# domargan/parallel-packed-csr

Hardware: AMD Instinct MI355X
Metric: edge-updates/sec (higher is better)
Workload: dtype u32; 1 GPU; config#2 1000000 random inserts on RMAT scale-20 / 10000000-edge core, 1 partition, labels raw; vertices=1048576, core_edges=10000000, parallelism=1 partition(s), 1 per GPU x 1 GPU(s), logN=32, distinct_update_batches=4, semantics=sequential stream order (bit-exact vs reference -threads=1)

## Files before the change

parallel-packed-csr_amd/csrc/engine.cc:

```cpp
#include "engine.h"

#include <stdio.h>
#include <stdlib.h>

#include <algorithm>
#include <map>
#include <memory>
#include <vector>
#include <chrono>

#include "gpu_rt.h"
#define GPU_DFREE(x) gpu::dfree_named((x), #x, __LINE__)
#include "pma_kernels.h"

namespace ppcsr {

#define GCHK(expr)                                                                       \
  do {                                                                                   \
    int _e = (expr);                                                                     \
    if (_e != 0) return fail(PPCSR_EHIP, std::string(#expr) + ": " + gpu::err_str(_e)); \
  } while (0)

struct DevGuard {
  std::vector<void **> slots;
// ... 41 lines not shown
  ChainTable *d_table = nullptr;
  unsigned long long *d_scan_state = nullptr;
  uint64_t scan_state_cap = 0, scan_nchunks = 0;
  Edge *d_scratch = nullptr;
  uint64_t scratch_cap = 0;
  int *d_nbr = nullptr;
  uint64_t nbr_cap = 0;
  uint32_t round = 0;
  uint32_t max_horizon = 4096, min_horizon = 64, rounds_per_sync = 32, init_horizon = 256;
  gpu::Timer timer;
  EngineStats st{};
  struct Snap {
    View v{};
    uint64_t cap_slots = 0, cap_nodes = 0;
    bool valid = false;
    uint32_t synced = 0;
    uint64_t gen = 0;
  };
  Snap snap, esnap;
  uint32_t snap_grid = 4096;
  bool snap_count = false;
  uint64_t snap_ctr[6] = {0, 0, 0, 0, 0, 0};
  unsigned long long *d_snapcnt = nullptr;
  uint64_t scc_ctr[8] = {0, 0, 0, 0, 0, 0, 0, 0};
  uint64_t msf_ctr[8] = {0, 0, 0, 0, 0, 0, 0, 0};
  uint32_t serial = 1;
  uint64_t array_gen = 1;
  bool stamps_clean = false;
  OptCtl *d_octl = nullptr, *h_octl = nullptr;
  uint32_t *d_vdbg = nullptr;
  uint32_t *d_status = nullptr, *d_carry0 = nullptr, *d_carry1 = nullptr;
  uint64_t carry_cap = 0, hslot_cap = 0;
  unsigned long long *d_regfail = nullptr, *d_pfail = nullptr;
  uint32_t *d_vws = nullptr, *d_vrs = nullptr;
  uint32_t *d_wstamp = nullptr, *d_rstamp = nullptr;
  uint32_t mode = 1;
  uint32_t epoch_ops = 1u << 20;
  uint32_t cur_epoch = 0;
  uint32_t epoch_short = 16384;
  uint32_t epoch_clean = 0, epoch_grow_after = 2;
  uint32_t epoch_adapt = 8, grow_eff = 2;
  uint64_t since_rollback = 0;
  double rb_dist = -1.0;
  uint32_t region_slots = 1024;
  uint32_t region_wide = 4096, region_calm = 8, region_eff = 0, region_clean = 0;
  uint32_t region_rare = 16384, region_rare_calm = 8, region_rare_dist = 65536;
  uint64_t region_rare_span = 0;
  uint32_t region_rare_cpr = 1536;
  double cpr_mean = -1.0;
  uint32_t resident_waves = 0;
  uint32_t opt_horizon = 6144;
  uint32_t start_horizon = 6144;
  uint32_t adaptive = 1;
  uint32_t rb_defer_table = 1u << 22;
  uint32_t scatter_blocks = 8192;
  uint32_t small_batch = 256;
  uint32_t excl_in_wave = 4096;
  uint32_t big_window = 32768, big_min = 256, big_grid = 64;
  dev::BigJob *d_jobs = nullptr;
  Edge *d_bigscratch = nullptr;
  uint64_t bigscratch_cap = 0;
  uint32_t rb_tile = 0;
  uint32_t rb_min_tiles = 4096;
  bool big_on = false;
  double big_rate = 0;
  bool check_lanes = true;
  uint32_t check_wave_chunks = 0;
  int check_force = -1;
  uint32_t rb_prefetch = 1;
  bool time_resize = false;
  double last_resize_ms = 0;
  uint32_t rb_bench_upper = 0;
  uint64_t rb_inplace_min = 1ull << 19;
  uint32_t rb_inplace_cpw = 0;
  uint32_t *d_ip = nullptr;
  uint32_t ip_epoch = 0;
  uint32_t ip_lists = 1;
  bool ip_used = false;
  uint32_t scatter_variant = 2;
  bool partial = false;
  bool profile = false;
  bool in_batch = false;
  uint32_t soft_barrier = 0;
  uint32_t defer_barrier = 0;
  uint32_t dbg_repeat = 0;
  uint32_t diag = 0;
// ... 12 lines not shown
    uint64_t rows_cap = 0;
    uint32_t *crow = nullptr, *ccnt = nullptr;
    unsigned long long *ooff = nullptr;
    uint64_t chunk_cap = 0;
    int *sdst = nullptr;
    uint32_t *sval = nullptr;
    uint64_t stage_cap = 0;
    unsigned long long *xs = nullptr;
    uint64_t xs_cap = 0;
  } q;
};

Engine::Engine() : p_(new Impl()) {}

static int ensure_plans(Engine::Impl &p) {
  const uint64_t need = (uint64_t)std::max(p.opt_horizon, p.max_horizon) + 64;
  if (p.plans_cap >= need) return 0;
  int e = gpu::sync(p.stream);
  if (e) return e;
  Plan *np = nullptr;
  if ((e = gpu::dmalloc((void **)&np, need * sizeof(Plan)))) return e;
  if (p.d_plans) GPU_DFREE(p.d_plans);
  p.d_plans = np;
  p.plans_cap = need;
  return 0;
}

static int reset_tags(Engine::Impl &p) {
  const uint64_t leaves = p.v.g.N >> p.v.g.sh;
  int e;
  if (p.v.wres && (e = gpu::dset(p.v.wres, 0xFF, leaves * sizeof(unsigned long long), p.stream))) return e;
  if (p.v.rres && (e = gpu::dset(p.v.rres, 0xFF, leaves * sizeof(unsigned long long), p.stream))) return e;
  if (p.v.dres && (e = gpu::dset(p.v.dres, 0xFF, leaves * sizeof(unsigned long long), p.stream))) return e;
  if (p.d_regfail && (e = gpu::dset(p.d_regfail, 0xFF, (leaves + 1) * sizeof(unsigned long long), p.stream))) return e;
  if (p.d_pfail && (e = gpu::dset(p.d_pfail, 0xFF, (leaves + 1) * sizeof(unsigned long long), p.stream))) return e;
  if (p.v.vw && (e = gpu::dset(p.v.vw, 0xFF, (p.n_cap + 1) * sizeof(unsigned long long), p.stream))) return e;
  if (p.v.vr && (e = gpu::dset(p.v.vr, 0xFF, (p.n_cap + 1) * sizeof(unsigned long long), p.stream))) return e;
  p.round = 0;
  return 0;
}

static int alloc_aux(Engine::Impl &p, View &v) {
  const uint64_t leaves = v.g.N >> v.g.sh;
  int e;
  if ((e = gpu::dmalloc((void **)&v.wres, leaves * sizeof(unsigned long long)))) return e;
  if ((e = gpu::dmalloc((void **)&v.rres, leaves * sizeof(unsigned long long)))) return e;
  if ((e = gpu::dmalloc((void **)&v.dres, leaves * sizeof(unsigned long long)))) return e;
  if ((e = gpu::dset(v.dres, 0xFF, leaves * sizeof(unsigned long long), p.stream))) return e;
  if ((e = gpu::dmalloc((void **)&p.d_wstamp, leaves * sizeof(uint32_t)))) return e;
  if ((e = gpu::dmalloc((void **)&p.d_rstamp, leaves * sizeof(uint32_t)))) return e;
  if ((e = gpu::dmalloc((void **)&p.d_regfail, (leaves + 1) * sizeof(unsigned long long)))) return e;
  if ((e = gpu::dmalloc((void **)&p.d_pfail, (leaves + 1) * sizeof(unsigned long long)))) return e;
  if ((e = gpu::dset(p.d_pfail, 0xFF, (leaves + 1) * sizeof(unsigned long long), p.stream))) return e;
  if ((e = gpu::dset(v.wres, 0xFF, leaves * sizeof(unsigned long long), p.stream))) return e;
  if ((e = gpu::dset(v.rres, 0xFF, leaves * sizeof(unsigned long long), p.stream))) return e;
  if ((e = gpu::dset(p.d_regfail, 0xFF, (leaves + 1) * sizeof(unsigned long long), p.stream))) return e;
  if ((e = gpu::dset(p.d_wstamp, 0, leaves * sizeof(uint32_t), p.stream))) return e;
  if ((e = gpu::dset(p.d_rstamp, 0, leaves * sizeof(uint32_t), p.stream))) return e;
  if ((e = gpu::dmalloc((void **)&v.ldirty, leaves * sizeof(uint32_t)))) return e;
  if ((e = gpu::dset(v.ldirty, 0, leaves * sizeof(uint32_t), p.stream))) return e;
  p.leaves_cap = leaves;
  p.round = 0;
  if (v.vw && (e = gpu::dset(v.vw, 0xFF, (p.n_cap + 1) * sizeof(unsigned long long), p.stream))) return e;
  if (v.vr && (e = gpu::dset(v.vr, 0xFF, (p.n_cap + 1) * sizeof(unsigned long long), p.stream))) return e;
  return 0;
}
static int alloc_vertex_aux(Engine::Impl &p, View &v) {
  const uint64_t cap = p.n_cap + 1;
  int e;
  if (v.vw) GPU_DFREE(v.vw);
  if (v.vr) GPU_DFREE(v.vr);
  if (p.d_vws) GPU_DFREE(p.d_vws);
  if (p.d_vrs) GPU_DFREE(p.d_vrs);
  if (v.vdirty) GPU_DFREE(v.vdirty);
  v.vw = v.vr = nullptr;
  v.vdirty = nullptr;
  p.d_vws = p.d_vrs = nullptr;
  if ((e = gpu::dmalloc((void **)&v.vdirty, cap * sizeof(uint32_t)))) return e;
  if ((e = gpu::dset(v.vdirty, 0, cap * sizeof(uint32_t), p.stream))) return e;
  if ((e = gpu::dmalloc((void **)&v.vw, cap * sizeof(unsigned long long)))) return e;
  if ((e = gpu::dmalloc((void **)&v.vr, cap * sizeof(unsigned long long)))) return e;
// ... 40 lines not shown
}

int Engine::create(uint32_t init_n, uint32_t src_n, int lock_search, int device, Engine **out, std::string *errmsg) {
  Engine *e = new Engine();
  int rc = e->init(init_n, src_n, lock_search, device);
  if (rc != PPCSR_OK) {
    if (errmsg) *errmsg = e->err_;
    e->p_->partial = true;
    delete e;
    *out = nullptr;
    return rc;
  }
  *out = e;
  return PPCSR_OK;
}

int Engine::init(uint32_t init_n, uint32_t src_n, int lock_search, int device) {
  Impl &p = *p_;
  device_ = device;
  int ndev = 0;
  GCHK(gpu::device_count(&ndev));
  if (ndev <= 0) return fail(PPCSR_EHIP, "no HIP device visible: the MI355X engine has no CPU fallback");
  if (device < 0 || device >= ndev) return fail(PPCSR_EINVAL, "bad device ordinal");
  GCHK(gpu::set_device(device));
  (void)gpu::last_error();
  GCHK(gpu::stream_create(&p.stream));
  GCHK(p.timer.init());
  {
    int cus = 0;
    GCHK(gpu::device_cus(device, &cus));
    if (cus > 0) {
      p.resident_waves = (uint32_t)cus * 28u;
      p.start_horizon = p.resident_waves;
      p.opt_horizon = 3u * p.resident_waves;
    }
  }
  const uint64_t N = initial_N(init_n, src_n);
  Geometry g;
  compute_geometry(N, src_n, lock_search, &g);
  p.v.g = g;
  p.v.big_window = kBigWindow;
  p.v.serial = p.serial;
  p.n_cap = std::max<uint64_t>(src_n, 16);
  p.leaves_cap = N >> g.sh;
  GCHK(gpu::dmalloc((void **)&p.v.items, N * sizeof(Edge)));
  GCHK(gpu::dmalloc((void **)&p.v.nodes, p.n_cap * sizeof(Node)));
  GCHK(gpu::dmalloc((void **)&p.v.leafcnt, p.leaves_cap * sizeof(uint32_t)));
  GCHK(alloc_aux(p, p.v));
  GCHK(alloc_vertex_aux(p, p.v));
  GCHK(gpu::dmalloc((void **)&p.d_octl, sizeof(OptCtl)));
  GCHK(gpu::hmalloc((void **)&p.h_octl, sizeof(OptCtl)));
  GCHK(gpu::dmalloc((void **)&p.d_ctl, sizeof(Control)));
  GCHK(gpu::hmalloc((void **)&p.h_ctl, sizeof(Control)));
  GCHK(gpu::dmalloc((void **)&p.d_stats, kStatShards * sizeof(StatShard)));
  GCHK(gpu::hmalloc((void **)&p.h_stats, kStatShards * sizeof(StatShard)));
  GCHK(gpu::dset(p.d_stats, 0, kStatShards * sizeof(StatShard), p.stream));
  GCHK(gpu::dmalloc((void **)&p.d_stats_snap, kStatShards * sizeof(StatShard)));
  GCHK(gpu::dmalloc((void **)&p.d_xout, sizeof(ExclOut)));
  GCHK(gpu::hmalloc((void **)&p.h_xout, sizeof(ExclOut)));
  GCHK(gpu::hmalloc((void **)&p.h_op1, sizeof(Op)));
  GCHK(gpu::dmalloc((void **)&p.d_total, 32 * sizeof(unsigned long long)));
  GCHK(gpu::hmalloc((void **)&p.h_total, sizeof(unsigned long long)));
  GCHK(gpu::dmalloc((void **)&p.d_table, sizeof(ChainTable)));
  GCHK(gpu::dmalloc((void **)&p.d_ip, (kIpHdrWords + 2 * (uint64_t)kIpMaxTiles) * sizeof(uint32_t)));
  GCHK(gpu::dset(p.d_ip, 0, (kIpHdrWords + 2 * (uint64_t)kIpMaxTiles) * sizeof(uint32_t), p.stream));
  {
    uint32_t *probe = p.d_ip + kIpHdrWords;
// ... 19 lines not shown

  std::vector<Node> nodes(src_n);
  {
    double index_d = 0.0;
    const double step = ((double)N) / src_n;
    for (uint32_t i = 0; i < src_n; i++) {
      nodes[i].beginning = (i == 0) ? 0u : nodes[i - 1].end;
      index_d += step;
      nodes[i].end = (uint32_t)(int)index_d;
      nodes[i].num_neighbors = 0;
    }
    if (src_n != 0) nodes[src_n - 1].end = (uint32_t)(N - 1);
  }
  if (src_n) {
    GCHK(gpu::h2d(p.v.nodes, nodes.data(), (uint64_t)src_n * sizeof(Node), p.stream));
    GCHK(gpu::sync(p.stream));
  }
  GPU_LAUNCH(p.stream, k_fill_null, grid_for(N * 3, 256 * 8), 256, p.v.items, (uint64_t)0, N);
  if (src_n) GPU_LAUNCH(p.stream, k_place_sentinels, grid_for(src_n, 256), 256, p.v);
  GPU_LAUNCH(p.stream, k_recount, grid_for((N + 63) / 64, 4), 256, p.v, (uint64_t)0, N);
  GCHK(gpu::sync(p.stream));
  GCHK(gpu::last_error());
  return PPCSR_OK;
}

Engine::~Engine() {
  Impl &p = *p_;
  gpu::set_device(device_);
  gpu::sync(p.stream);
  GPU_DFREE(p.v.items);
  GPU_DFREE(p.v.nodes);
  GPU_DFREE(p.v.leafcnt);
  free_aux(p, p.v);
  if (p.v.vw) GPU_DFREE(p.v.vw);
  if (p.v.vr) GPU_DFREE(p.v.vr);
  if (p.d_vws) GPU_DFREE(p.d_vws);
  if (p.d_vrs) GPU_DFREE(p.d_vrs);
  if (p.v.vdirty) GPU_DFREE(p.v.vdirty);
  GPU_DFREE(p.d_octl);
  gpu::hfree(p.h_octl);
  if (p.d_status) GPU_DFREE(p.d_status);
  if (p.d_vdbg) GPU_DFREE(p.d_vdbg);
  if (p.d_carry0) GPU_DFREE(p.d_carry0);
  if (p.d_carry1) GPU_DFREE(p.d_carry1);
  GPU_DFREE(p.d_ctl);
  gpu::hfree(p.h_ctl);
  GPU_DFREE(p.d_stats);
  gpu::hfree(p.h_stats);
  GPU_DFREE(p.d_stats_snap);
  GPU_DFREE(p.d_xout);
  gpu::hfree(p.h_xout);
  gpu::hfree(p.h_op1);
  GPU_DFREE(p.d_total);
  gpu::hfree(p.h_total);
  GPU_DFREE(p.d_table);
  if (p.d_ip) GPU_DFREE(p.d_ip);
  if (p.d_snapcnt) GPU_DFREE(p.d_snapcnt);
  GPU_DFREE(p.d_plans);
  if (p.d_ops) GPU_DFREE(p.d_ops);
  if (p.d_rank) GPU_DFREE(p.d_rank);
  if (p.d_tiles) GPU_DFREE(p.d_tiles);
  if (p.d_nbr) GPU_DFREE(p.d_nbr);
  if (p.d_scratch) GPU_DFREE(p.d_scratch);
  if (p.d_scan_state) GPU_DFREE(p.d_scan_state);
  if (p.d_jobs) GPU_DFREE(p.d_jobs);
  if (p.d_bigscratch) GPU_DFREE(p.d_bigscratch);
// ... 48 lines not shown
  if (k == "region_slots") {
    if (value < 1 || (value & (value - 1))) return fail(PPCSR_EINVAL, "region_slots must be a power of two");
    p.region_slots = (uint32_t)value;
    p.region_eff = 0;
    return PPCSR_OK;
  }
  if (k == "region_wide") {
    if (value < 1 || (value & (value - 1))) return fail(PPCSR_EINVAL, "region_wide must be a power of two");
    p.region_wide = (uint32_t)value;
    return PPCSR_OK;
  }
  if (k == "region_rare") {
    if (value < 0 || (value & (value - 1))) return fail(PPCSR_EINVAL, "region_rare must be 0 or a power of two");
    p.region_rare = (uint32_t)value;
    return PPCSR_OK;
  }
  if (k == "region_rare_calm") {
    p.region_rare_calm = (uint32_t)std::max<int64_t>(1, value);
    return PPCSR_OK;
  }
  if (k == "region_rare_cpr") {
    p.region_rare_cpr = (uint32_t)std::max<int64_t>(0, value);
    return PPCSR_OK;
  }
  if (k == "region_rare_dist") {
    p.region_rare_dist = (uint32_t)std::max<int64_t>(1, value);
    return PPCSR_OK;
  }
  if (k == "region_calm") {
    p.region_calm = (uint32_t)std::max<int64_t>(1, value);
    return PPCSR_OK;
  }
  if (k == "opt_horizon") {
    if (value < 1 || value > (1 << 20)) return fail(PPCSR_EINVAL, "opt_horizon out of range");
    p.opt_horizon = (uint32_t)value;
    gpu::set_device(device_);
    GCHK(ensure_plans(p));
    p.start_horizon = std::min<uint32_t>(p.start_horizon, p.opt_horizon);
    if (!p.adaptive) p.start_horizon = p.opt_horizon;
    return PPCSR_OK;
  }
  if (k == "scatter_blocks") {
    p.scatter_blocks = (uint32_t)std::max<int64_t>(64, value);
    return PPCSR_OK;
  }
  if (k == "search_narrow") {
    p.v.g.narrow = value ? 1u : 0u;
    return PPCSR_OK;
  }
  if (k == "small_batch") {
    p.small_batch = value < 0 ? 0u : (uint32_t)value;
    return PPCSR_OK;
  }
  if (k == "excl_in_wave") {
    p.excl_in_wave = (uint32_t)std::max<int64_t>(64, value);
    return PPCSR_OK;
  }
  if (k == "big_window") {
    if (value < 64 || (value & (value - 1))) return fail(PPCSR_EINVAL, "big_window must be a power of two >= 64");
    p.big_window = (uint32_t)std::min<int64_t>(value, 1 << 20);
    return PPCSR_OK;
  }
  if (k == "big_min") {
    p.big_min = (uint32_t)std::max<int64_t>(64, std::min<int64_t>(value, kBigWindow));
    return PPCSR_OK;
  }
  if (k == "big_grid") {
    p.big_grid = (uint32_t)std::max<int64_t>(1, std::min<int64_t>(value, 256));
    return PPCSR_OK;
  }
  if (k == "rb_tile") {
    uint32_t t = 0;
    if (value > 0) for (t = 8; t < (uint32_t)value && t < kRbTile; t <<= 1) {}
    p.rb_tile = t;
// ... 21 lines not shown
    p.snap_grid = (uint32_t)value;
    return PPCSR_OK;
  }
  if (k == "snap_count") {
    if (value && !p.d_snapcnt) {
      gpu::set_device(device_);
      GCHK(gpu::dmalloc((void **)&p.d_snapcnt, 2 * sizeof(unsigned long long)));
    }
    p.snap_count = value != 0;
    return PPCSR_OK;
  }
  if (k == "rb_inplace_cpw") {
    p.rb_inplace_cpw = value >= 16 ? 16u : (value >= 8 ? 8u : 0u);
    return PPCSR_OK;
  }
  if (k == "rb_inplace_min") {
    p.rb_inplace_min = value < 0 ? 0ull : (uint64_t)value;
    return PPCSR_OK;
  }
  if (k == "check_lanes") {
    p.check_force = value < 0 ? -1 : (value ? 1 : 0);
    return PPCSR_OK;
  }
  if (k == "rb_bench_upper") {
    p.rb_bench_upper = value ? 1u : 0u;
    return PPCSR_OK;
  }
  if (k == "rb_prefetch") {
    p.rb_prefetch = value ? 1u : 0u;
    return PPCSR_OK;
  }
  if (k == "scatter_variant") {
    p.scatter_variant = value > 2 ? 2u : (uint32_t)value;
    return PPCSR_OK;
  }
  if (k == "adaptive") {
    p.adaptive = value != 0;
    return PPCSR_OK;
  }
  if (k == "resident_waves") {
    if (value < 0 || value > (1 << 20)) return fail(PPCSR_EINVAL, "resident_waves out of range");
    p.resident_waves = (uint32_t)value;
    return PPCSR_OK;
  }
  if (k == "start_horizon") {
    if (value < 1 || value > (1 << 20)) return fail(PPCSR_EINVAL, "start_horizon out of range");
    p.start_horizon = (uint32_t)value;
    return PPCSR_OK;
  }
  if (k == "test_block_rebalance") {
    const uint64_t ws = (uint64_t)value >> 32, wl = (uint64_t)value & 0xFFFFFFFFull;
    if (wl < 64 || (wl & (wl - 1)) || ws % wl || ws + wl > p.v.g.N || (wl >> p.v.g.sh) > dev::kBigLeaves) return fail(PPCSR_EINVAL, "bad window");
    gpu::set_device(device_);
    Edge *sc = nullptr;
    GCHK(gpu::dmalloc((void **)&sc, wl * sizeof(Edge)));
    GPU_LAUNCH(p.stream, k_block_rebalance, 1, dev::kBigThreads, p.v, ws, wl, sc);
    GCHK(gpu::sync(p.stream));
    GCHK(gpu::last_error());
    gpu::dfree(sc);
    return PPCSR_OK;
  }
  if (k == "marker") {
    gpu::set_device(device_);
    uint32_t *np_ = nullptr;
    switch (value) {
      case 0: GPU_LAUNCH(p.stream, k_mark_0, 1, 64, np_); break;
// ... 253 lines not shown
  const uint32_t kEpochShort = p.epoch_short;
  if (p.cur_epoch == 0 || p.cur_epoch > p.epoch_ops) p.cur_epoch = p.epoch_ops;
  while (e0 < n) {
    uint64_t e1 = std::min<uint64_t>(e0 + p.cur_epoch, n);
    if (forced_e1 > e0 && forced_e1 < e1) e1 = forced_e1;
    if (p.round > 0xFFFF0000u) GCHK(reset_tags(p));
    GCHK(snap_commit(p, p.esnap));
    GCHK(gpu::d2d(p.d_stats_snap, p.d_stats, kStatShards * sizeof(StatShard), p.stream));
    if (!p.stamps_clean) {
      const uint64_t leaves = p.v.g.N >> p.v.g.sh;
      GCHK(gpu::dset(p.d_wstamp, 0, leaves * sizeof(uint32_t), p.stream));
      GCHK(gpu::dset(p.d_rstamp, 0, leaves * sizeof(uint32_t), p.stream));
      GCHK(gpu::dset(p.d_vws, 0, (p.n_cap + 1) * sizeof(uint32_t), p.stream));
      GCHK(gpu::dset(p.d_vrs, 0, (p.n_cap + 1) * sizeof(uint32_t), p.stream));
      p.stamps_clean = true;
    }
    OptCtl &c = *p.h_octl;
    memset(&c, 0, sizeof(c));
    const uint32_t pp0 = p.round & 1u;
    c.hor[pp0] = 0;
    c.used[pp0] = 0;
    c.nf[pp0] = (uint32_t)e0;
    c.adaptive = p.adaptive;
    c.cur_h[pp0] = p.adaptive ? std::min(p.start_horizon, p.opt_horizon) : p.opt_horizon;
    c.book_round = p.round;
    for (int t = 0; t < 3; t++) {
      c.minkept[t] = kMax;
      c.gbar[t] = c.sbar[t] = ~0ull;
    }
    c.e1 = (uint32_t)e1;
    c.max_horizon = p.opt_horizon;
    c.width_cap = p.opt_horizon;
    c.resident = p.resident_waves;
    c.viol_idx = kMax;
    c.skip_idx = kMax;
    c.skip_round = 0;
    GCHK(gpu::h2d(p.d_octl, p.h_octl, sizeof(OptCtl), p.stream));
    int rs = 0;
    if (p.region_eff < p.region_slots) p.region_eff = p.region_slots;
    while ((p.region_eff >> rs) > (uint32_t)p.v.g.logN) rs++;
    bool epoch_open = true;
    uint32_t cur_width = c.cur_h[pp0];
    uint64_t carry_now = 0;
    unsigned long long jobs_seen = 0, rounds_seen = 0, planned_seen = 0, long_seen = 0;
    uint64_t chunk_pending = e1 - e0;
    double chunk_cpr = 0.9 * (double)std::min<uint64_t>(cur_width, e1 - e0);
    unsigned long long prev_rounds = 0, prev_committed = 0;
    uint32_t excl_cooldown = 0;
    while (epoch_open) {
      OptArgs a;
      a.v = p.v;
      a.v.big_window = use_big ? bigw : kBigWindow;
      a.big_min = p.big_min;
      a.jobs = use_big ? p.d_jobs : (dev::BigJob *)nullptr;
      a.bigscratch = p.d_bigscratch;
      a.bigscratch_stride = bigw;
      a.ops = d_ops;
      a.plans = p.d_plans;
      a.status = p.d_status;
      a.vdbg = p.d_vdbg;
      a.carry0 = p.d_carry0;
      a.carry1 = p.d_carry1;
      a.carry_cap = (uint32_t)p.carry_cap;
      a.ctl = p.d_octl;
      a.stats = p.d_stats;
      a.regfail = p.d_regfail;
      a.pfail = p.d_pfail;
      a.wstamp = p.d_wstamp;
      a.rstamp = p.d_rstamp;
      a.vws = p.d_vws;
      a.vrs = p.d_vrs;
      a.regshift = rs;
      a.diag = p.diag;
      a.defer_barrier = p.defer_barrier;
      const bool extras = p.diag != 0 || p.dbg_repeat != 0;
      a.dbg = p.dbg_repeat;
      a.dg = p.diag >= 2 ? p.d_dg : (uint32_t *)nullptr;
      a.soft_barrier = p.soft_barrier ? p.soft_barrier : a.v.big_window / 2u;
      if (!p.soft_barrier && p.region_rare_span && p.region_eff >= p.region_rare) a.soft_barrier = 0x40000000u;
      uint32_t gh = p.opt_horizon;
      {
        const uint64_t want = std::max<uint64_t>(1024, 4ull * (cur_width ? cur_width : p.opt_horizon));
        if (want < gh) gh = (uint32_t)want;
        const uint64_t pend = (chunk_pending + 255) & ~255ull;
        if (pend < gh) gh = (uint32_t)std::max<uint64_t>(pend, 256);
        const uint64_t need = (carry_now + 255) & ~255ull;
        if (gh < need) gh = (uint32_t)std::min<uint64_t>(need, p.opt_horizon);
      }
      const uint32_t blocks = (gh + 3) / 4;
      if (gh != c.max_horizon) {
        GCHK(gpu::h2d(&p.d_octl->max_horizon, &gh, sizeof(uint32_t), p.stream));
        c.max_horizon = gh;
      }
      uint32_t rounds = p.rounds_per_sync;
      {
        const double per_round = std::max(1.0, 0.85 * chunk_cpr);
        const double est = (double)chunk_pending / per_round + 2.0;
        if (est < (double)rounds) rounds = (uint32_t)std::max(2.0, est);
      }
      if (excl_cooldown) {
        rounds = std::min<uint32_t>(rounds, 8u);
        excl_cooldown--;
      }
      if (p.profile && p.events.size() < 5ull * rounds) {
        const size_t oldn = p.events.size();
        p.events.resize(5ull * rounds);
        for (size_t i = oldn; i < p.events.size(); i++) GCHK(p.events[i].init());
      }
      for (uint32_t r = 0; r < rounds; r++) {
        a.round = ++p.round;
        if (p.profile) p.events[5 * r + 0].record(p.stream);
        if (extras) GPU_LAUNCH(p.stream, o_plan_x, blocks, 256, a); else GPU_LAUNCH(p.stream, o_plan, blocks, 256, a);
        if (p.profile) p.events[5 * r + 1].record(p.stream);
        if (extras) GPU_LAUNCH(p.stream, o_check_x, blocks, 256, a);
        else if (p.check_force >= 0 ? p.check_force == 1 : p.check_lanes) GPU_LAUNCH(p.stream, o_check, (gh + kCkThreads - 1) / kCkThreads, kCkThreads, a);
        else GPU_LAUNCH(p.stream, o_check_w, blocks, 256, a);
        if (p.profile) p.events[5 * r + 2].record(p.stream);
        if (extras) GPU_LAUNCH(p.stream, o_apply_x, blocks, 256, a); else GPU_LAUNCH(p.stream, o_apply, blocks, 256, a);
        if (p.profile) p.events[5 * r + 3].record(p.stream);
        if (use_big && p.big_on) GPU_LAUNCH(p.stream, o_big, p.big_grid, 1024, a);
        if (p.profile) p.events[5 * r + 4].record(p.stream);
      }
      {
        a.round = p.round + 1;
        GPU_LAUNCH(p.stream, o_settle, 1, 64, a);
      }
      GCHK(gpu::d2h(p.h_octl, p.d_octl, sizeof(OptCtl), p.stream));
      GCHK(gpu::sync(p.stream));
      GCHK(gpu::last_error());
      if (p.profile) {
        for (uint32_t r = 0; r < rounds; r++) {
// ... 1717 lines not shown
```

parallel-packed-csr_amd/csrc/pma_spec_rounds.h:

```cpp
#pragma once
#include "pma_rounds.h"

namespace ppcsr {

constexpr uint32_t kStripes = 8;
struct OptCtl {
  uint32_t hor[2];
  uint32_t used[2];
  uint32_t nf[2];
  uint32_t cur_h[2];
  uint32_t kept[3][kStripes];
  uint32_t minkept[3];
  unsigned long long gbar[3];
  unsigned long long sbar[3];
  uint32_t njobs[3];
  uint32_t e1;
  uint32_t violation, excl, done, error;
  uint32_t max_horizon, excl_idx;
  uint32_t excl_later;
  uint32_t width_cap;
  uint32_t resident;
  uint32_t viol_idx;
  uint32_t adaptive;
  uint32_t book_round;
  uint32_t need_big;
  uint32_t big_done_round;
  unsigned long long jobs_total;
  unsigned long long long_checks;
  uint32_t skip_idx, skip_round;
  unsigned long long rounds, committed, planned;
  uint32_t viol_info[8];
  unsigned long long why[12];
};
struct OptArgs {
  View v;
  const Op *ops;
  Plan *plans;
  uint32_t *status, *vdbg;
  uint32_t *carry0, *carry1;
  uint32_t carry_cap;
  OptCtl *ctl;
  StatShard *stats;
  unsigned long long *regfail;
  unsigned long long *pfail;
  uint32_t *wstamp, *rstamp;
  uint32_t *vws, *vrs;
  uint32_t round;
  int regshift;
  uint32_t diag;
  uint32_t dbg;
  uint32_t defer_barrier;
  uint32_t soft_barrier;
  uint32_t big_min;
  dev::BigJob *jobs;
  Edge *bigscratch;
  uint32_t bigscratch_stride;
  uint32_t *dg;
};
constexpr uint32_t kBigJobs = 256;
constexpr uint32_t kRegionPadLeaves = 2u;
constexpr uint32_t kGrowLeaves = 8u;
constexpr uint32_t OS_PASS = 1u, OS_STAMP_BAD = 2u;


PMA_DEV bool key_earlier(unsigned long long k, uint32_t tag, uint32_t idx) { return (uint32_t)(k >> 32) == tag && (uint32_t)k < idx; }

using dev::PlanHead;
using dev::kHeadRanges;
#define PMA_FOR_EACH_READ_LEAF_H(h, pl, lane, LEAFVAR, BODY)                                  \
  do {                                                                                        \
    if ((h).nr <= (uint32_t)kHeadRanges && (h).nlong == 0u) {                                 \
      if ((uint32_t)(lane) < (h).nr)                                                          \
        for (uint32_t LEAFVAR = (h).my_lo; LEAFVAR <= (h).my_hi; LEAFVAR++) { BODY; }         \
    } else {                                                                                  \
      PMA_FOR_EACH_READ_LEAF(pl, lane, LEAFVAR, BODY);                                        \
    }                                                                                         \
  } while (0)

struct RoundState {
  uint32_t hor, used, nf, ch;
  uint32_t pre[kStripes + 1];
  uint32_t done, excl, excl_idx, excl_later, error, need_big;
  uint32_t prev_hor, prev_committed, prev_jobs;
};
PMA_DEV RoundState round_begin(const OptArgs &a, const OptCtl *c) {
  const uint32_t r = a.round, pp = (r - 1u) & 1u, pt = (r - 1u) % 3u;
  const uint32_t p_hor = c->hor[pp], p_used = c->used[pp], p_nf = c->nf[pp], p_ch = c->cur_h[pp];
  const uint32_t e1 = c->e1, max_h = c->max_horizon, wcap = c->width_cap, res = c->resident, adaptive = c->adaptive;
  const unsigned long long gb = c->gbar[pt];
  const uint32_t minkept = c->minkept[pt];
  const uint32_t p_jobs = c->njobs[pt], big_done = c->big_done_round;
  RoundState s;
  uint32_t K = 0;
#pragma unroll
  for (uint32_t q = 0; q < kStripes; q++) {
    s.pre[q] = K;
    K += c->kept[pt][q];
  }
  s.pre[kStripes] = K;
  const uint32_t ncommitted = p_hor - K;
  const uint32_t new_nf = p_nf + (p_hor - p_used);
  uint32_t ch = p_ch ? p_ch : wcap;
  if (adaptive && p_hor >= ch && p_hor > 0u) {
    if (res && ch >= res) {
      if (ncommitted * 100u > p_hor * 85u) ch += res;
      else if (ch > res && ncommitted * 100u < p_hor * 70u) ch -= res;
      else if (ch == res && ncommitted * 100u < p_hor * 10u) ch -= ch / 4u;
    } else {
      if (ncommitted * 100u > p_hor * 30u) ch += ch / 4u;
      else if (ncommitted * 100u < p_hor * 10u) ch -= ch / 4u;
      if (res && ch > res) ch = res;
    }
  }
  if (res && ch > res) ch -= ch % res;
  if (ch < 1024u) ch = 1024u;
  if (ch > wcap) ch = wcap;
  const uint32_t avail = e1 - new_nf, room = ch > K ? ch - K : 0u;
  uint32_t nh = K + (avail < room ? avail : room);
  if (nh > max_h) nh = max_h;
  s.error = K > max_h ? 1u : 0u;
  s.hor = nh;
  s.used = K;
  s.nf = new_nf;
  s.ch = ch;
  s.done = (K == 0u && new_nf == e1) ? 1u : 0u;
  const uint32_t lowest = K ? minkept : new_nf;
  const uint32_t tag = (uint32_t)(make_key(r - 1u, 0) >> 32);
  s.excl = (!s.done && (uint32_t)(gb >> 32) == tag && (uint32_t)gb == lowest) ? 1u : 0u;
  s.excl_idx = lowest;
  s.excl_later = (K >= 1u && new_nf - lowest - 1u > K - 1u) ? 1u : 0u;
  s.prev_hor = p_hor;
  s.prev_committed = ncommitted;
  s.prev_jobs = p_jobs;
  s.need_big = (p_hor > 0u && p_jobs > 0u && big_done != r - 1u) ? 1u : 0u;
  return s;
}
PMA_DEV void round_record(const OptArgs &a, OptCtl *c, const RoundState &s) {
  const uint32_t r = a.round, par = r & 1u, nt = (r + 1u) % 3u;
  if (c->book_round != r - 1u) {
// ... 84 lines not shown
  } else {
    idx = wv::bcast(rw, RW_NF) + (wid - used);
  }
  const uint32_t skip_idx = wv::bcast(rw, RW_SKIP_IDX), skip_round = wv::bcast(rw, RW_SKIP_ROUND);
  Op op = a.ops[idx];
  op.src = wv::uni(op.src);
  op.dst = wv::uni(op.dst);
  op.op = wv::uni(op.op);
  Plan *pl = &a.plans[wid];
  if (a.round == skip_round && idx == skip_idx) {
    dev::store_plan_header(pl, K_SKIP, 0, 0, 0, 0, 1, 0, 1, 0, 0, 0, 0, 0, 0, 0, 0, idx, op);
    return;
  }
  if (EXTRAS && (a.dbg & 1u)) (void)dev::plan_op(a.v, op, pl, idx);
  if (EXTRAS && (a.dbg & 2u) && op.src < a.v.g.n) {
    dev::RangeRec rr2;
    dev::SearchHit h2;
    const Node nd = a.v.nodes[op.src];
    const uint32_t r = dev::pma_search(a.v, op.dst, nd.beginning + 1u, nd.end, rr2, &h2);
    if (r == 0xFFFFFFF0u) a.status[wid] = rr2.nr + h2.known;
  }
  if (EXTRAS && (a.dbg & 4u)) {
    const RoundState r2 = round_begin(a, c);
    if (r2.hor == 0xFFFFFFF0u) a.status[wid] = r2.nf;
  }
  const dev::PlanRegs pr = dev::plan_op(a.v, op, pl, idx);
  const unsigned long long key = make_key(a.round, idx);
  const uint32_t kind = pr.kind;
  if (kind == K_EXCL) {
    if (lane == 0) wv::atomic_min_u64(&c->gbar[rt], key);
    return;
  }
  if (kind == K_DUP) {
    if (lane == 0) wv::atomic_min_u64(&a.v.dres[pr.wleaf_lo], key);
  } else if (kind_strong(kind)) {
    const uint32_t wl = pr.wleaf_lo, wh = pr.wleaf_hi;
    for (uint32_t base = wl; base <= wh; base += 64) {
      const uint32_t leaf = base + (uint32_t)lane;
      if (leaf <= wh) wv::atomic_min_u64(&a.v.wres[leaf], key);
    }
    if ((pr.wlen >= a.soft_barrier || (a.defer_barrier && wid < used && pr.wlen >= a.defer_barrier)) && lane == 0) {
      wv::atomic_min_u64(&c->sbar[rt], key);
    }
    const uint32_t ml = pr.mv_lo, mh = pr.mv_hi;
    if (ml <= mh)
      for (uint64_t base = ml; base <= (uint64_t)mh; base += 64) {
        const uint64_t u = base + (uint64_t)lane;
        if (u <= (uint64_t)mh) wv::atomic_min_u64(&a.v.vw[u], key);
      }
  }
  if (pr.nlong == 0u) {
    if ((uint32_t)lane < pr.nr)
      for (uint32_t leaf = pr.my_lo; leaf <= pr.my_hi; leaf++) wv::atomic_min_u64(&a.v.rres[leaf], key);
  } else {
    wv::fence();
    PMA_FOR_EACH_READ_LEAF(pl, lane, leaf, wv::atomic_min_u64(&a.v.rres[leaf], key));
  }
  if (kind_real(kind) && op.src < a.v.g.n) {
    if (lane == 0 && (pr.sdep & 1u)) wv::atomic_min_u64(&a.v.vr[op.src], key);
    if (lane == 1 && (pr.sdep & 2u) && op.src + 1u < a.v.g.n) wv::atomic_min_u64(&a.v.vr[op.src + 1u], key);
  }
}
PMA_KERNEL void PMA_LAUNCH_BOUNDS(256, 8) o_plan(OptArgs a) { o_plan_t<false>(a); }
PMA_KERNEL void o_plan_x(OptArgs a) { o_plan_t<true>(a); }

template <bool EXTRAS>
PMA_DEV void o_check_one(const OptArgs &a, OptCtl *c, uint32_t par, uint32_t wid, const PlanHead &h, const Plan *pl, unsigned long long gbar,
                         unsigned long long sbar) {
  const int lane = wv::lane();
  const uint32_t idx = h.idx;
  const uint32_t kind = h.kind;
  const unsigned long long key = make_key(a.round, idx);
  const uint32_t tag = (uint32_t)(key >> 32);
  bool fail = (kind == K_EXCL) || key_earlier(gbar, tag, idx) || key_earlier(sbar, tag, idx);
  uint32_t why = (kind == K_EXCL) ? 0u : (fail ? 1u : 99u);
  if (fail) {
    if ((EXTRAS && a.diag) && lane == 0) wv::atomic_add_u64(&c->why[why], 1ull);
    if (lane == 0 && (EXTRAS && a.diag) && a.dg != nullptr) {
      uint32_t *r = a.dg + 4ull * idx;
      r[0] += 1u;
      r[1] = why;
      r[2] = (kind == K_EXCL) ? idx : (uint32_t)(key_earlier(gbar, tag, idx) ? gbar : sbar);
      r[3] = h.wlen;
    }
    if (lane == 0) a.status[wid] = 0u;
    return;
  }
#define PMA_WHY(code) do { if ((EXTRAS && a.diag) && (code) < why) why = (code); } while (0)
#define PMA_WHYB(code, bkey) do { if ((EXTRAS && a.diag) && (code) < why) { why = (code); blk = (uint32_t)(bkey); } } while (0)
  uint32_t blk = kMax;
  bool stamp_bad = false;
  const uint32_t me1 = idx + 1u;
  const bool writes = kind_writes(kind);
  const bool strong = kind_strong(kind);
  if (kind == K_DUP) {
    const uint32_t leaf = h.wleaf_lo;
    if (key_earlier(a.v.wres[leaf], tag, idx)) { fail = true; PMA_WHY(2u); }
    if (a.v.dres[leaf] != key) { fail = true; PMA_WHY(2u); }
  }
  if (strong) {
    const uint32_t wl = h.wleaf_lo, wh = h.wleaf_hi;
    for (uint32_t base = wl; base <= wh; base += 256u) {
      unsigned long long kw[4], kd[4], kr[4];
      uint32_t sw[4], sr[4];
#pragma unroll
      for (int q = 0; q < 4; q++) {
        const uint32_t leaf = base + (uint32_t)q * 64u + (uint32_t)lane;
        const bool in = leaf <= wh && leaf >= base;
        kw[q] = in ? a.v.wres[leaf] : key;
        kd[q] = in ? a.v.dres[leaf] : ~0ull;
        kr[q] = in ? a.v.rres[leaf] : ~0ull;
        sw[q] = in ? a.wstamp[leaf] : 0u;
        sr[q] = in ? a.rstamp[leaf] : 0u;
      }
#pragma unroll
      for (int q = 0; q < 4; q++) {
        const uint32_t leaf = base + (uint32_t)q * 64u + (uint32_t)lane;
        if (kw[q] != key) { fail = true; PMA_WHYB(3u, kw[q]); }
        if (key_earlier(kd[q], tag, idx)) { fail = true; PMA_WHYB(2u, kd[q]); }
        if (key_earlier(kr[q], tag, idx)) { fail = true; PMA_WHYB(4u, kr[q]); }
        if (sw[q] > me1 || sr[q] > me1) {
          stamp_bad = true;
          a.vdbg[4 * wid + 0] = leaf;
          a.vdbg[4 * wid + 1] = sw[q] > me1 ? sw[q] : sr[q];
          a.vdbg[4 * wid + 2] = sw[q] > me1 ? 1u : 2u;
        }
      }
      if (wh - base < 256u) break;
    }
  }
  PMA_FOR_EACH_READ_LEAF_H(h, pl, lane, leaf, {
// ... 119 lines not shown
  const bool writes = kind_writes(kind), strong = kind_strong(kind), real = kind_real(kind);
  const int sh = a.v.g.sh;
  const uint32_t nleaves = (uint32_t)(a.v.g.N >> sh);
  const bool barred = (kind == K_EXCL) || key_earlier(gbar, tag, idx) || key_earlier(sbar, tag, idx);
  uint32_t ll = writes ? wl : (index >> sh), lh = writes ? wh : ll;
  ll = (ll > kRegionPadLeaves) ? ll - kRegionPadLeaves : 0u;
  lh = (lh + kRegionPadLeaves < nleaves) ? lh + kRegionPadLeaves : nleaves - 1u;
  const uint32_t pglo = ll >> a.regshift, pghi = lh >> a.regshift;
  uint32_t wleaves = writes && wlen ? (wlen >> sh) : 1u;
  if (wleaves < 1u) wleaves = 1u;
  uint32_t gblk = wleaves * 4u;
  if (gblk < kGrowLeaves) gblk = kGrowLeaves;
  const uint32_t anchor = writes && wlen ? (wstart >> sh) : (index >> sh);
  uint32_t bl = anchor & ~(gblk - 1u), bh = bl + gblk - 1u;
  if (ll < bl) bl = ll;
  if (lh > bh) bh = lh;
  if (bh >= nleaves) bh = nleaves - 1u;
  bool longr = false;
#pragma unroll
  for (int r = 0; r < kCkRanges; r++)
    if ((uint32_t)r < nr && rhi[r] - rlo[r] >= 2u) longr = true;
  const bool moves = strong && mv_lo <= mv_hi;
  const bool complex = active && !barred && real &&
                       (nlong != 0u || nr > (uint32_t)kCkRanges || longr || (writes && wh - wl >= kCkWrite) || (moves && mv_hi - mv_lo >= kCkMovedMax) ||
                        bh - bl >= kCkMark || pghi - pglo >= 4u);
  const bool mine = active && !barred && !complex;
  bool fail = barred, stamp_bad = false;
  uint32_t bad_where = 0, bad_stamp = 0, bad_what = 0;
  {
    const bool wany = mine && writes;
    const uint32_t w0 = wany ? wl : 0u, w1 = (wany && wh > wl) ? wh : w0;
    const unsigned long long kw0 = a.v.wres[w0], kd0 = a.v.dres[w0], kr0 = a.v.rres[w0], kw1 = a.v.wres[w1], kd1 = a.v.dres[w1], kr1 = a.v.rres[w1];
    const uint32_t sw0 = a.wstamp[w0], sr0 = a.rstamp[w0], sw1 = a.wstamp[w1], sr1 = a.rstamp[w1];
    unsigned long long rk[kCkRanges][2];
    uint32_t rs[kCkRanges][2], rl[kCkRanges][2];
#pragma unroll
    for (int r = 0; r < kCkRanges; r++) {
      const bool on = mine && (uint32_t)r < nr;
      rl[r][0] = on ? rlo[r] : 0u;
      rl[r][1] = on ? rhi[r] : 0u;
      rk[r][0] = a.v.wres[rl[r][0]];
      rk[r][1] = a.v.wres[rl[r][1]];
      rs[r][0] = a.wstamp[rl[r][0]];
      rs[r][1] = a.wstamp[rl[r][1]];
    }
    const bool vany = mine && real && src < a.v.g.n;
    const bool von0 = vany && (sdep & 1u), von1 = vany && (sdep & 2u) && src + 1u < a.v.g.n;
    const uint32_t u0 = von0 ? src : 0u, u1 = von1 ? src + 1u : 0u;
    const unsigned long long kv0 = a.v.vw[u0], kv1 = a.v.vw[u1];
    const uint32_t sv0 = a.vws[u0], sv1 = a.vws[u1];
    const bool many = vany && moves;
    unsigned long long mk[kCkMoved];
    uint32_t m1[kCkMoved], m2[kCkMoved], mu[kCkMoved];
#pragma unroll
    for (uint32_t q = 0; q < kCkMoved; q++) {
      mu[q] = (many && mv_lo + q <= mv_hi) ? mv_lo + q : 0u;
      mk[q] = a.v.vr[mu[q]];
      m1[q] = a.vrs[mu[q]];
      m2[q] = a.vws[mu[q]];
    }
    if (mine && kind == K_DUP) {
      if (key_earlier(kw0, tag, idx)) fail = true;
      if (kd0 != key) fail = true;
    }
    if (mine && strong) {
      if (kw0 != key || kw1 != key) fail = true;
      if (key_earlier(kd0, tag, idx) || key_earlier(kd1, tag, idx)) fail = true;
      if (key_earlier(kr0, tag, idx) || key_earlier(kr1, tag, idx)) fail = true;
      if (sw1 > me1 || sr1 > me1) {
        stamp_bad = true;
        bad_where = w1;
        bad_stamp = sw1 > me1 ? sw1 : sr1;
        bad_what = sw1 > me1 ? 1u : 2u;
      }
      if (sw0 > me1 || sr0 > me1) {
        stamp_bad = true;
        bad_where = w0;
        bad_stamp = sw0 > me1 ? sw0 : sr0;
        bad_what = sw0 > me1 ? 1u : 2u;
      }
    }
#pragma unroll
    for (int r = 0; r < kCkRanges; r++) {
      if (mine && (uint32_t)r < nr) {
#pragma unroll
        for (int e = 0; e < 2; e++) {
          if (key_earlier(rk[r][e], tag, idx)) fail = true;
          if (rs[r][e] > me1) {
            stamp_bad = true;
            bad_where = rl[r][e];
            bad_stamp = rs[r][e];
            bad_what = 3u;
          }
        }
      }
    }
// ... 278 lines not shown
```

Before: 281.9 million edge-updates/s.

## Hash duplicate-op claims into a side table and tune adaptive horizon widening

```diff
diff --git a/parallel-packed-csr_amd/csrc/engine.cc b/parallel-packed-csr_amd/csrc/engine.cc
--- a/parallel-packed-csr_amd/csrc/engine.cc
+++ b/parallel-packed-csr_amd/csrc/engine.cc
@@ -97,6 +97,8 @@
   uint32_t *d_status = nullptr, *d_carry0 = nullptr, *d_carry1 = nullptr;
   uint64_t carry_cap = 0, hslot_cap = 0;
   unsigned long long *d_regfail = nullptr, *d_pfail = nullptr;
+  unsigned long long *d_ddup = nullptr;
+  uint32_t ddup_size = 1u << 18;
   uint32_t *d_vws = nullptr, *d_vrs = nullptr;
   uint32_t *d_wstamp = nullptr, *d_rstamp = nullptr;
   uint32_t mode = 1;
@@ -117,6 +119,7 @@
   uint32_t opt_horizon = 6144;
   uint32_t start_horizon = 6144;
   uint32_t adaptive = 1;
+  uint32_t wide_from = 3, wide_up = 950, wide_down = 900;
   uint32_t rb_defer_table = 1u << 22;
   uint32_t scatter_blocks = 8192;
   uint32_t small_batch = 256;
@@ -195,6 +198,7 @@
   if (p.v.wres && (e = gpu::dset(p.v.wres, 0xFF, leaves * sizeof(unsigned long long), p.stream))) return e;
   if (p.v.rres && (e = gpu::dset(p.v.rres, 0xFF, leaves * sizeof(unsigned long long), p.stream))) return e;
   if (p.v.dres && (e = gpu::dset(p.v.dres, 0xFF, leaves * sizeof(unsigned long long), p.stream))) return e;
+  if (p.d_ddup && (e = gpu::dset(p.d_ddup, 0xFF, (uint64_t)p.ddup_size * sizeof(unsigned long long), p.stream))) return e;
   if (p.d_regfail && (e = gpu::dset(p.d_regfail, 0xFF, (leaves + 1) * sizeof(unsigned long long), p.stream))) return e;
   if (p.d_pfail && (e = gpu::dset(p.d_pfail, 0xFF, (leaves + 1) * sizeof(unsigned long long), p.stream))) return e;
   if (p.v.vw && (e = gpu::dset(p.v.vw, 0xFF, (p.n_cap + 1) * sizeof(unsigned long long), p.stream))) return e;
@@ -210,6 +214,8 @@
   if ((e = gpu::dmalloc((void **)&v.rres, leaves * sizeof(unsigned long long)))) return e;
   if ((e = gpu::dmalloc((void **)&v.dres, leaves * sizeof(unsigned long long)))) return e;
   if ((e = gpu::dset(v.dres, 0xFF, leaves * sizeof(unsigned long long), p.stream))) return e;
+  if (!p.d_ddup && (e = gpu::dmalloc((void **)&p.d_ddup, (uint64_t)p.ddup_size * sizeof(unsigned long long)))) return e;
+  if ((e = gpu::dset(p.d_ddup, 0xFF, (uint64_t)p.ddup_size * sizeof(unsigned long long), p.stream))) return e;
   if ((e = gpu::dmalloc((void **)&p.d_wstamp, leaves * sizeof(uint32_t)))) return e;
   if ((e = gpu::dmalloc((void **)&p.d_rstamp, leaves * sizeof(uint32_t)))) return e;
   if ((e = gpu::dmalloc((void **)&p.d_regfail, (leaves + 1) * sizeof(unsigned long long)))) return e;
@@ -316,7 +322,7 @@
     if (cus > 0) {
       p.resident_waves = (uint32_t)cus * 28u;
       p.start_horizon = p.resident_waves;
-      p.opt_horizon = 3u * p.resident_waves;
+      p.opt_horizon = 4u * p.resident_waves;
     }
   }
   const uint64_t N = initial_N(init_n, src_n);
@@ -402,6 +408,7 @@
   GPU_DFREE(p.v.nodes);
   GPU_DFREE(p.v.leafcnt);
   free_aux(p, p.v);
+  if (p.d_ddup) GPU_DFREE(p.d_ddup);
   if (p.v.vw) GPU_DFREE(p.v.vw);
   if (p.v.vr) GPU_DFREE(p.v.vr);
   if (p.d_vws) GPU_DFREE(p.d_vws);
@@ -516,6 +523,7 @@
     return PPCSR_OK;
   }
   if (k == "opt_horizon") {
+    static_assert((1ull << 20) * 1000ull < (1ull << 32), "opt_horizon bound against round_begin's 32-bit per-mille compares");
     if (value < 1 || value > (1 << 20)) return fail(PPCSR_EINVAL, "opt_horizon out of range");
     p.opt_horizon = (uint32_t)value;
     gpu::set_device(device_);
@@ -524,6 +532,18 @@
     if (!p.adaptive) p.start_horizon = p.opt_horizon;
     return PPCSR_OK;
   }
+  if (k == "ddup_size") {
+    if (value < 1 || value > (1 << 24) || (value & (value - 1))) return fail(PPCSR_EINVAL, "ddup_size must be a power of two <= 2^24");
+    gpu::set_device(device_);
+    GCHK(gpu::sync(p.stream));
+    unsigned long long *nt = nullptr;
+    GCHK(gpu::dmalloc((void **)&nt, (uint64_t)value * sizeof(unsigned long long)));
+    if (p.d_ddup) GPU_DFREE(p.d_ddup);
+    p.d_ddup = nt;
+    p.ddup_size = (uint32_t)value;
+    GCHK(gpu::dset(p.d_ddup, 0xFF, (uint64_t)p.ddup_size * sizeof(unsigned long long), p.stream));
+    return PPCSR_OK;
+  }
   if (k == "scatter_blocks") {
     p.scatter_blocks = (uint32_t)std::max<int64_t>(64, value);
     return PPCSR_OK;
@@ -611,6 +631,11 @@
   }
   if (k == "scatter_variant") {
     p.scatter_variant = value > 2 ? 2u : (uint32_t)value;
+    return PPCSR_OK;
+  }
+  if (k == "wide_from" || k == "wide_up" || k == "wide_down") {
+    if (value < 0 || value > 1000) return fail(PPCSR_EINVAL, k + " out of range");
+    (k == "wide_from" ? p.wide_from : k == "wide_up" ? p.wide_up : p.wide_down) = (uint32_t)value;
     return PPCSR_OK;
   }
   if (k == "adaptive") {
@@ -930,6 +955,9 @@
     c.max_horizon = p.opt_horizon;
     c.width_cap = p.opt_horizon;
     c.resident = p.resident_waves;
+    c.wide_from = p.wide_from;
+    c.wide_up = p.wide_up;
+    c.wide_down = p.wide_down;
     c.viol_idx = kMax;
     c.skip_idx = kMax;
     c.skip_round = 0;
@@ -944,6 +972,7 @@
     uint64_t chunk_pending = e1 - e0;
     double chunk_cpr = 0.9 * (double)std::min<uint64_t>(cur_width, e1 - e0);
     unsigned long long prev_rounds = 0, prev_committed = 0;
+    bool long_epoch = false;
     uint32_t excl_cooldown = 0;
     while (epoch_open) {
       OptArgs a;
@@ -964,6 +993,8 @@
       a.stats = p.d_stats;
       a.regfail = p.d_regfail;
       a.pfail = p.d_pfail;
+      a.ddup = p.d_ddup;
+      a.ddup_mask = p.ddup_size - 1u;
       a.wstamp = p.d_wstamp;
       a.rstamp = p.d_rstamp;
       a.vws = p.d_vws;
@@ -980,6 +1011,10 @@
       {
         const uint64_t want = std::max<uint64_t>(1024, 4ull * (cur_width ? cur_width : p.opt_horizon));
         if (want < gh) gh = (uint32_t)want;
+        if (p.resident_waves && p.wide_from) {
+          const uint32_t soft = std::max<uint32_t>(cur_width, p.wide_from * p.resident_waves);
+          if (soft < gh) gh = soft;
+        }
         const uint64_t pend = (chunk_pending + 255) & ~255ull;
         if (pend < gh) gh = (uint32_t)std::max<uint64_t>(pend, 256);
         const uint64_t need = (carry_now + 255) & ~255ull;
@@ -995,6 +1030,8 @@
         const double per_round = std::max(1.0, 0.85 * chunk_cpr);
         const double est = (double)chunk_pending / per_round + 2.0;
         if (est < (double)rounds) rounds = (uint32_t)std::max(2.0, est);
+        if (long_epoch) rounds = std::max<uint32_t>(rounds, std::max<uint32_t>(2u, p.rounds_per_sync / 4u));
+        if (rounds == p.rounds_per_sync) long_epoch = true;
       }
       if (excl_cooldown) {
         rounds = std::min<uint32_t>(rounds, 8u);
diff --git a/parallel-packed-csr_amd/csrc/pma_spec_rounds.h b/parallel-packed-csr_amd/csrc/pma_spec_rounds.h
--- a/parallel-packed-csr_amd/csrc/pma_spec_rounds.h
+++ b/parallel-packed-csr_amd/csrc/pma_spec_rounds.h
@@ -22,6 +22,7 @@
   uint32_t resident;
   uint32_t viol_idx;
   uint32_t adaptive;
+  uint32_t wide_from, wide_up, wide_down;
   uint32_t book_round;
   uint32_t need_big;
   uint32_t big_done_round;
@@ -45,6 +46,8 @@
   unsigned long long *pfail;
   uint32_t *wstamp, *rstamp;
   uint32_t *vws, *vrs;
+  unsigned long long *ddup;
+  uint32_t ddup_mask;
   uint32_t round;
   int regshift;
   uint32_t diag;
@@ -87,6 +90,7 @@
   const uint32_t r = a.round, pp = (r - 1u) & 1u, pt = (r - 1u) % 3u;
   const uint32_t p_hor = c->hor[pp], p_used = c->used[pp], p_nf = c->nf[pp], p_ch = c->cur_h[pp];
   const uint32_t e1 = c->e1, max_h = c->max_horizon, wcap = c->width_cap, res = c->resident, adaptive = c->adaptive;
+  const uint32_t wfrom = c->wide_from, wup = c->wide_up, wdown = c->wide_down;
   const unsigned long long gb = c->gbar[pt];
   const uint32_t minkept = c->minkept[pt];
   const uint32_t p_jobs = c->njobs[pt], big_done = c->big_done_round;
@@ -103,8 +107,10 @@
   uint32_t ch = p_ch ? p_ch : wcap;
   if (adaptive && p_hor >= ch && p_hor > 0u) {
     if (res && ch >= res) {
-      if (ncommitted * 100u > p_hor * 85u) ch += res;
-      else if (ch > res && ncommitted * 100u < p_hor * 70u) ch -= res;
+      const bool top = wfrom && ch >= wfrom * res;
+      const uint32_t up = top ? wup : 850u, down = (wfrom && ch > wfrom * res) ? wdown : 700u;
+      if (ncommitted * 1000u > p_hor * up) ch += res;
+      else if (ch > res && ncommitted * 1000u < p_hor * down) ch -= res;
       else if (ch == res && ncommitted * 100u < p_hor * 10u) ch -= ch / 4u;
     } else {
       if (ncommitted * 100u > p_hor * 30u) ch += ch / 4u;
@@ -255,7 +261,10 @@
     return;
   }
   if (kind == K_DUP) {
-    if (lane == 0) wv::atomic_min_u64(&a.v.dres[pr.wleaf_lo], key);
+    if (lane == 0) {
+      wv::atomic_min_u64(&a.v.dres[pr.wleaf_lo], key);
+      wv::atomic_min_u64(&a.ddup[pr.index & a.ddup_mask], key);
+    }
   } else if (kind_strong(kind)) {
     const uint32_t wl = pr.wleaf_lo, wh = pr.wleaf_hi;
     for (uint32_t base = wl; base <= wh; base += 64) {
@@ -319,7 +328,7 @@
   if (kind == K_DUP) {
     const uint32_t leaf = h.wleaf_lo;
     if (key_earlier(a.v.wres[leaf], tag, idx)) { fail = true; PMA_WHY(2u); }
-    if (a.v.dres[leaf] != key) { fail = true; PMA_WHY(2u); }
+    if (a.ddup[h.index & a.ddup_mask] != key) { fail = true; PMA_WHY(2u); }
   }
   if (strong) {
     const uint32_t wl = h.wleaf_lo, wh = h.wleaf_hi;
@@ -505,6 +514,7 @@
     const uint32_t w0 = wany ? wl : 0u, w1 = (wany && wh > wl) ? wh : w0;
     const unsigned long long kw0 = a.v.wres[w0], kd0 = a.v.dres[w0], kr0 = a.v.rres[w0], kw1 = a.v.wres[w1], kd1 = a.v.dres[w1], kr1 = a.v.rres[w1];
     const uint32_t sw0 = a.wstamp[w0], sr0 = a.rstamp[w0], sw1 = a.wstamp[w1], sr1 = a.rstamp[w1];
+    const unsigned long long kt = a.ddup[(wany && kind == K_DUP) ? (index & a.ddup_mask) : 0u];
     unsigned long long rk[kCkRanges][2];
     uint32_t rs[kCkRanges][2], rl[kCkRanges][2];
 #pragma unroll
@@ -534,7 +544,7 @@
     }
     if (mine && kind == K_DUP) {
       if (key_earlier(kw0, tag, idx)) fail = true;
-      if (kd0 != key) fail = true;
+      if (kt != key) fail = true;
     }
     if (mine && strong) {
       if (kw0 != key || kw1 != key) fail = true;
```

Result: faster. 298.6 million edge-updates/s (median of 6 runs) (+5.9%).
